# zachramsey/pm-rl

Hardware: AMD Instinct MI355X
Metric: env-steps/sec (whole node) at 65k envs x 30 assets; reward MAE vs CPU ref (higher is better)
Workload: dtype f64

## Files before the change

pm-rl_amd/csrc/step_relay.h:

```cpp
#pragma once
#include "env_step.h"
#include "scalar_vec.h"

namespace pmenv_dev {

struct RelayParams {
    uint32_t scal;
    uint32_t epoch;
    uint64_t* w;
    uint64_t* list;
    uint32_t* done;
    uint32_t spin;
    uint32_t rot;
    uint32_t grid;
    const int32_t* kp_in;
    int32_t* kp_out;
    const float* halo_in;
    float* halo_out;
    uint32_t* seq;
    int32_t* kp;
    float* halo;
    uint32_t B;
    uint32_t halo_stride;
    const float* obs;
    uint32_t par;
};
enum { kSeqD = 0, kSeqE = 1, kSeqV = 2, kSeqC = 3, kSeqEC = 4, kSeqHobs = 6 };

struct RelayCtx {
    uint32_t epoch;
    const int32_t* kp_in;
    int32_t* kp_out;
    const float* halo_in;
    float* halo_out;
};
template <bool SEQ>
__device__ __forceinline__ RelayCtx relay_ctx(const RelayParams& r) {
    RelayCtx c{r.epoch, r.kp_in, r.kp_out, r.halo_in, r.halo_out};
    if constexpr (SEQ) {
        const uint32_t par = __builtin_amdgcn_readfirstlane(r.seq[kSeqC]);
        c.epoch = __builtin_amdgcn_readfirstlane(r.seq[kSeqEC]);
        c.kp_in = r.kp + (size_t)par * r.B;
        c.kp_out = r.kp + (size_t)(par ^ 1u) * r.B;
        c.halo_in = r.halo + (size_t)par * r.halo_stride;
        c.halo_out = r.halo + (size_t)(par ^ 1u) * r.halo_stride;
    }
    return c;
}

struct KArgs {
    StepParams p;
    RelayParams r;
    uint32_t qtot;
};
__device__ __forceinline__ KArgs kargs() {
    typedef __attribute__((address_space(4))) const uint32_t KWord;
    KWord* ka = (KWord*)__builtin_amdgcn_kernarg_segment_ptr();
    asm volatile("" : "+s"(ka));
    uint32_t w[sizeof(KArgs) / 4];
#pragma unroll
    for (size_t i = 0; i < sizeof(KArgs) / 4; ++i) w[i] = ka[i];
    KArgs k;
    __builtin_memcpy(&k, w, sizeof(KArgs));
    return k;
}

constexpr uint32_t kStampSlots = 16, kStampMaxWg = 40960;
static __device__ uint64_t* g_relay_stamps;
template <bool ST, bool DRAIN = false>
__device__ __forceinline__ uint64_t relay_clock(uint32_t dep) {
    uint64_t t = 0;
    if constexpr (ST) {
        if constexpr (DRAIN)
            asm volatile("s_waitcnt vmcnt(0)\n\ts_memrealtime %0\n\ts_waitcnt lgkmcnt(0)" : "=s"(t) : "v"(dep) : "memory");
        else
            asm volatile("s_memrealtime %0\n\ts_waitcnt lgkmcnt(0)" : "=s"(t) : "v"(dep) : "memory");
    }
    return t;
}
template <bool ST, int K>
__device__ __forceinline__ void relay_stamps_put(uint32_t bid, uint32_t epoch, const uint64_t (&ts)[K]) {
    if constexpr (ST) {
        uint64_t* s = g_relay_stamps;
        if (s && threadIdx.x == 0 && bid < kStampMaxWg) {
#pragma unroll
            for (int k = 0; k < K; ++k) s[((size_t)(epoch % kStampSlots) * kStampMaxWg + bid) * 8 + k] = ts[k];
        }
    }
}

__device__ __forceinline__ void relay_put(uint64_t* w, uint32_t epoch, uint32_t bits) {
    __hip_atomic_store(w, ((uint64_t)epoch << 32) | bits, __ATOMIC_RELAXED, __HIP_MEMORY_SCOPE_AGENT);
}
__device__ __forceinline__ uint64_t relay_get(const uint64_t* w) {
    return __hip_atomic_load(const_cast<uint64_t*>(w), __ATOMIC_RELAXED, __HIP_MEMORY_SCOPE_AGENT);
}

__device__ __forceinline__ uint32_t relay_list_read(const RelayParams& r, uint32_t epoch) {
    __atomic_signal_fence(__ATOMIC_SEQ_CST);
    __builtin_amdgcn_s_waitcnt(0);
    __atomic_signal_fence(__ATOMIC_SEQ_CST);
    const uint64_t lw = relay_get(r.list);
    return (uint32_t)(lw >> 32) == epoch ? (uint32_t)lw : 0u;
}

template <int BLOCK, int KL, int KA, bool ST = false>
__device__ __forceinline__ uint32_t relay_scalar(const StepParams& p, const RelayParams& r, int s, uint32_t epoch,
                                                 int32_t* kp_out, uint64_t t_entry = 0) {
    uint64_t ts[3] = {t_entry, 0, 0};
    constexpr int EPW = 64 / KL, EPB = (BLOCK / 64) * EPW;
    const int lane = threadIdx.x & 63;
    const int b = s * EPB + (int)(threadIdx.x >> 6) * EPW + lane / KL;
    const int j = lane % KL;
    const int N = p.N;
    const bool env_ok = b < p.B;
    uint32_t listed;
    if constexpr (KA == 0) {
        const ScalarIn in = scalar_load<KL>(p, b, lane);
        const ScalarMid m = scalar_core<KL>(p, b, lane, in);
        if (env_ok && j < N) relay_put(r.w + (size_t)b * N + j, epoch, __float_as_uint(m.wp));
        if (env_ok && j == 0) kp_out[b] = m.k + 1;
        listed = relay_list_read(r, epoch);
        ts[1] = relay_clock<ST>(listed);
        scalar_tail<KL>(p, b, lane, in, m);
    } else {
        const VecIn<KA> in = vec_load<KL, KA, true>(p, b, lane);
        const VecMid<KA> m = vec_core<KL, KA, true>(p, b, lane, in);
#pragma unroll
        for (int e = 0; e < KA; ++e) {
            const int n = j + e * KL;
            if (env_ok && n < N) relay_put(r.w + (size_t)b * N + n, epoch, __float_as_uint(m.wp[e]));
        }
        if (env_ok && j == 0) kp_out[b] = in.k + 1;
        listed = relay_list_read(r, epoch);
        ts[1] = relay_clock<ST>(listed);
        vec_tail<KL, KA, true>(p, b, lane, in, m);
    }
    ts[2] = relay_clock<ST, true>(0);
    relay_stamps_put<ST>((uint32_t)s, epoch, ts);
    return listed;
}

template <int BLOCK, int V, int POL, bool OUT, bool ADOPT, bool ST = false>
__device__ __forceinline__ bool relay_tile(const StepParams& p, const RelayParams& r, uint32_t qtot, uint32_t spin, uint32_t t,
                                           uint32_t epoch, const int32_t* kp_in, const float* halo_in,
                                           float* halo_out, f4* sh4, f4* sh_bar, float* sh_wp, int32_t* sh_kc,
                                           int32_t* sh_ok, uint64_t t_entry = 0) {
    uint64_t ts[6] = {t_entry, 0, 0, 0, 0, 0};
    constexpr int kAux = POL == 1 ? 2 : 0;
    constexpr int CPW = BLOCK * V, F = 5;
    const int tid = threadIdx.x, lane = tid & 63, wave = tid >> 6;
    const uint32_t c0 = t * CPW;
    const uint32_t nblk = min((uint32_t)CPW, qtot - c0);
    const auto rs = make_rsrc(p.obs + (size_t)c0 * 4, nblk * 16u);
    f4 own[V];
#pragma unroll
    for (int v = 0; v < V; ++v) own[v] = buf_load4<kAux>(rs, (uint32_t)(64 * V * wave + 64 * v + lane) * 16u);
    const uint32_t ntiles = (qtot + CPW - 1) / CPW;
    const uint32_t nh = t + 1 < ntiles ? min(2u, qtot - c0 - nblk) : 0u;
    const float* hsrc = OUT ? p.obs + (size_t)(c0 + nblk) * 4 : halo_in + (size_t)t * 8;
    const f4 hal = buf_load4<0>(make_rsrc(hsrc, nh * 16u), tid < 2 ? (uint32_t)tid * 16u : 0xFFFFFFF0u);
    __builtin_amdgcn_sched_barrier(0);
    const int N = p.N, W = p.W, WF = W * F;
    const uint32_t per4 = (uint32_t)(N * WF) >> 2;
    const uint32_t b_lo = fdiv(c0, p.div_units);
    const uint32_t g_lo = b_lo * (uint32_t)N + fdiv(4u * (c0 - b_lo * per4), p.div_wf);
    const uint32_t ql = c0 + nblk - 1u;
    const uint32_t b_hi = fdiv(ql, p.div_units);
    const uint32_t g_hi = b_hi * (uint32_t)N + fdiv(4u * (ql - b_hi * per4) + 3u, p.div_wf);
    const bool mine = (uint32_t)tid <= g_hi - g_lo;
    const uint32_t g = g_lo + (mine ? (uint32_t)tid : 0u);
    const uint32_t b = g / (uint32_t)N, n = g - b * (uint32_t)N;
    const float* barb = env_bar(p, (int)b);
    const float nanv = __int_as_float(0x7fc00000);
    f4 xb = f4{nanv, nanv, nanv, nanv};
    int32_t kc = 0;
    uint64_t ww = 0;
    if (barb) xb = *reinterpret_cast<const f4*>(barb + (size_t)n * 4);
    kc = kp_in[b];
    ww = relay_get(r.w + g);
    bool ready = !mine || (uint32_t)(ww >> 32) == epoch;
    ts[1] = relay_clock<ST>((uint32_t)ww);
    for (uint32_t polls = 0; !ADOPT && !__all(ready) && polls < spin; ++polls) {
        __builtin_amdgcn_s_sleep(2);
        if (!ready) {
            ww = relay_get(r.w + g);
            ready = (uint32_t)(ww >> 32) == epoch;
        }
    }
    const bool wave_ok = __all(ready);
    ts[2] = relay_clock<ST>((uint32_t)ww);
    if (mine) {
        sh_bar[tid] = xb;
        sh_wp[tid] = __uint_as_float((uint32_t)ww);
        sh_kc[tid] = kc;
    }
#pragma unroll
    for (int v = 0; v < V; ++v) sh4[64 * V * wave + 64 * v + lane] = own[v];
    if (tid < 2) sh4[CPW + tid] = hal;
    if (lane == 0) sh_ok[wave] = wave_ok ? 1 : 0;
    __syncthreads();
    ts[3] = relay_clock<ST>(0);
    if constexpr (ADOPT) {
        bool tile_ok = true;
#pragma unroll
        for (int w = 0; w < BLOCK / 64; ++w) tile_ok = tile_ok && sh_ok[w] != 0;
        if (!tile_ok) return false;
        if (tid == 0)
            sh_ok[BLOCK / 64] = __hip_atomic_exchange(r.done + t, epoch, __ATOMIC_RELAXED, __HIP_MEMORY_SCOPE_AGENT) != epoch;
        __syncthreads();
        if (!sh_ok[BLOCK / 64]) return true;
    }
    const auto rd = OUT ? make_rsrc(p.obs_out + (size_t)c0 * 4, nblk * 16u) : rs;
    const bool first_out = !OUT && t > 0;
    bool ok = true;
#pragma unroll
    for (int v = 0; v < V; ++v) {
        const int j = 64 * V * wave + 64 * v + lane;
        const uint32_t q = min(c0 + (uint32_t)j, qtot - 1u);
        const uint32_t bq = fdiv(q, p.div_units);
        const uint32_t j0 = 4u * (q - bq * per4);
        const uint32_t row = fdiv(j0, p.div_wf);
        const int kk = (int)(j0 - row * (uint32_t)WF);
        const int i = (int)(bq * (uint32_t)N + row - g_lo);
        const f4 n1 = sh4[j + 1], n2 = sh4[j + 2];
        const float sh[4] = {n1.y, n1.z, n1.w, n2.x};
        const float un[4] = {own[v].x, own[v].y, own[v].z, own[v].w};
        f4 o = compose2(p, kk, sh_kc[i], un, sh, [&](f4& x, float& xwp) {
            x = sh_bar[i];
            xwp = sh_wp[i];
        });
        if (!ADOPT && v == 0) {
            int32_t okv = 1;
#pragma unroll
            for (int w = 0; w < BLOCK / 64; ++w) okv &= sh_ok[w];
            ok = __builtin_amdgcn_readfirstlane(okv) != 0;
        }
        buf_store4<kAux>(rd, ok ? (uint32_t)j * 16u : 0x80000000u, o);
        if (ok && first_out && j < 2) reinterpret_cast<f4*>(halo_out)[2 * (t - 1) + j] = o;
    }
    ts[4] = relay_clock<ST>(0);
    ts[5] = relay_clock<ST, true>(0);
    relay_stamps_put<ST>(r.scal + t, epoch, ts);
    return ok;
}

template <int BLOCK, int V, int POL, bool OUT, bool SEQ>
__device__ __forceinline__ void relay_adopt(f4* sh4, f4* sh_bar, float* sh_wp, int32_t* sh_kc, int32_t* sh_ok,
                                            uint32_t listed) {
    constexpr int kB = BLOCK / 64 + 1;
    const int wave = threadIdx.x >> 6;
    if ((threadIdx.x & 63) == 0) sh_ok[wave] = (int32_t)__builtin_amdgcn_readfirstlane(listed);
    __syncthreads();
    uint32_t n = 0;
#pragma unroll
    for (int w = 0; w < BLOCK / 64; ++w) n = max(n, (uint32_t)sh_ok[w]);
    if (n == 0) return;
    const KArgs ka = kargs();
    const RelayCtx c = relay_ctx<SEQ>(ka.r);
    for (uint32_t i = 0; i < n; ++i) {
        __syncthreads();
        if (threadIdx.x == 0) {
            const uint64_t e = relay_get(ka.r.list + 1 + i);
            int32_t t = (uint32_t)(e >> 32) == c.epoch ? (int32_t)(uint32_t)e : -1;
            if (t >= 0 && __hip_atomic_load(ka.r.done + t, __ATOMIC_RELAXED, __HIP_MEMORY_SCOPE_AGENT) == c.epoch)
                t = -1;
            sh_ok[kB] = t;
        }
        __syncthreads();
        const int32_t t = __builtin_amdgcn_readfirstlane(sh_ok[kB]);
        if (t >= 0)
            (void)relay_tile<BLOCK, V, POL, OUT, true>(ka.p, ka.r, ka.qtot, 0u, (uint32_t)t, c.epoch, c.kp_in, c.halo_in,
                                                       c.halo_out, sh4, sh_bar, sh_wp, sh_kc, sh_ok);
    }
}

template <int BLOCK, int V, int POL, bool OUT, bool SEQ>
__device__ __forceinline__ void relay_defer(uint32_t t, f4* sh4, f4* sh_bar, float* sh_wp, int32_t* sh_kc,
                                            int32_t* sh_ok) {
    const KArgs ka = kargs();
    const RelayCtx c = relay_ctx<SEQ>(ka.r);
    if (threadIdx.x == 0) {
        uint64_t lw = relay_get(ka.r.list), nw;
        do {
            nw = (uint32_t)(lw >> 32) == c.epoch ? lw + 1 : ((uint64_t)c.epoch << 32) | 1u;
        } while (!__hip_atomic_compare_exchange_strong(ka.r.list, &lw, nw, __ATOMIC_RELAXED, __ATOMIC_RELAXED,
                                                        __HIP_MEMORY_SCOPE_AGENT));
        const uint32_t slot = (uint32_t)(lw >> 32) == c.epoch ? (uint32_t)lw : 0u;
        relay_put(ka.r.list + 1 + slot, c.epoch, t);
        __atomic_signal_fence(__ATOMIC_SEQ_CST);
        __builtin_amdgcn_s_waitcnt(0);
        __atomic_signal_fence(__ATOMIC_SEQ_CST);
    }
    __syncthreads();
    (void)relay_tile<BLOCK, V, POL, OUT, true>(ka.p, ka.r, ka.qtot, 0u, t, c.epoch, c.kp_in, c.halo_in, c.halo_out, sh4,
                                               sh_bar, sh_wp, sh_kc, sh_ok);
}

template <int BLOCK, int V, int POL, bool OUT, int KL, int KA, int OCC = 1, bool SEQ = false, int ANY = 0>
__global__ __launch_bounds__(BLOCK) __attribute__((amdgpu_waves_per_eu(OCC))) void step_relay_kernel(
    StepParams p, RelayParams r, uint32_t qtot) {
    __shared__ f4 sh4[BLOCK * V + 2];
    __shared__ f4 sh_bar[BLOCK];
    __shared__ float sh_wp[BLOCK];
    __shared__ int32_t sh_kc[BLOCK];
    __shared__ int32_t sh_ok[BLOCK / 64 + 2];
    const RelayCtx c = relay_ctx<SEQ>(r);
    if constexpr (SEQ) {
        if (blockIdx.x == 0 && threadIdx.x == 0) {
            const uint64_t hobs = OUT ? 0ull : (uint64_t)(uintptr_t)r.obs;
            r.seq[kSeqD] = (uint32_t)((c.kp_in - r.kp) / r.B) ^ 1u;
            r.seq[kSeqE] = c.epoch;
            r.seq[kSeqV] = 1u;
            r.seq[kSeqHobs] = (uint32_t)hobs;
            r.seq[kSeqHobs + 1] = (uint32_t)(hobs >> 32);
        }
    }
    constexpr bool kSt = ANY == 2;
    const uint64_t t_entry = relay_clock<kSt>(0);
    uint32_t bid = blockIdx.x;
    if constexpr (ANY == 1) {
        bid += r.rot;
        if (bid >= r.grid) bid -= r.grid;
    }
    if (bid < r.scal) {
        const uint32_t listed = relay_scalar<BLOCK, KL, KA, kSt>(p, r, (int)bid, c.epoch, c.kp_out, t_entry);
        relay_adopt<BLOCK, V, POL, OUT, SEQ>(sh4, sh_bar, sh_wp, sh_kc, sh_ok, listed);
    } else if (!relay_tile<BLOCK, V, POL, OUT, false, kSt>(p, r, qtot, ANY == 1 ? r.spin : kRelaySpin, bid - r.scal, c.epoch,
                                                           c.kp_in, c.halo_in, c.halo_out, sh4, sh_bar, sh_wp, sh_kc,
                                                           sh_ok, t_entry)) {
        relay_defer<BLOCK, V, POL, OUT, SEQ>(bid - r.scal, sh4, sh_bar, sh_wp, sh_kc, sh_ok);
    }
}

static __global__ __launch_bounds__(256) void relay_prime_kernel(StepParams p, RelayParams r, int prime_kp, int seq) {
    uint32_t d = r.par;
    bool kp = prime_kp != 0, halo = p.halo != nullptr;
    if (seq) {
        d = __builtin_amdgcn_readfirstlane(r.seq[kSeqD]);
        const uint32_t e = __builtin_amdgcn_readfirstlane(r.seq[kSeqE]);
        const uint32_t v = __builtin_amdgcn_readfirstlane(r.seq[kSeqV]);
        const uint64_t hobs = (uint64_t)__builtin_amdgcn_readfirstlane(r.seq[kSeqHobs]) |
                              ((uint64_t)__builtin_amdgcn_readfirstlane(r.seq[kSeqHobs + 1]) << 32);
        kp = v == 0;
        halo = halo && (v == 0 || hobs != (uint64_t)(uintptr_t)p.obs);
        if (blockIdx.x == 0 && threadIdx.x == 0) {
            r.seq[kSeqC] = d;
            r.seq[kSeqEC] = e + 1u == 0u ? 1u : e + 1u;
        }
    }
    if (halo) {
        p.halo += (size_t)d * r.halo_stride;
        copy_halo(p);
    }
    if (kp) {
        int32_t* kpd = r.kp + (size_t)d * r.B;
        for (int b = blockIdx.x * blockDim.x + threadIdx.x; b < p.B; b += gridDim.x * blockDim.x) kpd[b] = p.k[b];
    }
}

}
```

Baseline: 104.5 million.

## Compose relay observation tiles via shared-memory image shift when rows share a mode

Each tile now votes on whether all its rows are in shift mode or full-ring mode, packing the mode bits with the readiness flag in the shared vote word. When the modes agree, the new bar and weight values are scattered into the shared-memory image, and each output chunk becomes a plain shifted read, or in full mode a phase-selected blend. This replaces the per-element division and compose2 call. Mixed tiles fall back to the old per-element path. It adds an extra __syncthreads and index arithmetic that is easy to get wrong.

```diff
diff --git a/pm-rl_amd/csrc/compose_shift.h b/pm-rl_amd/csrc/compose_shift.h
--- /dev/null
+++ b/pm-rl_amd/csrc/compose_shift.h
@@ -0,0 +1,33 @@
+#pragma once
+#include <stdint.h>
+
+#if defined(__HIPCC__)
+#define PMENV_SHIFT_HD __host__ __device__ inline
+#else
+#define PMENV_SHIFT_HD inline
+#endif
+
+namespace pmenv_shift {
+
+constexpr int kF = 5;
+enum { kModeShift = 1, kModeFull = 2 };
+
+PMENV_SHIFT_HD int32_t image_floats(int cpw) { return 4 * (cpw + 2); }
+PMENV_SHIFT_HD bool in_image(int32_t cell, int cpw) { return cell >= 0 && cell < image_floats(cpw); }
+
+PMENV_SHIFT_HD int row_mode(bool storage, int32_t k, int W) { return storage && k >= W - 1 ? kModeFull : kModeShift; }
+PMENV_SHIFT_HD bool rows_mixed(int votes) { return votes == (kModeShift | kModeFull); }
+
+PMENV_SHIFT_HD int32_t ring_slot(int32_t k, int W) { return (int32_t)(((uint32_t)k + 1u) % (uint32_t)W); }
+
+PMENV_SHIFT_HD int32_t src_cell(int32_t row_off, int WF, int e) { return row_off + WF + e; }
+PMENV_SHIFT_HD int32_t slot_cell(int32_t row_off, int32_t slot) { return row_off + slot * kF + (kF - 1); }
+
+PMENV_SHIFT_HD uint32_t chunk_phase(uint32_t q) { return (4u * (q % (uint32_t)kF)) % (uint32_t)kF; }
+PMENV_SHIFT_HD uint32_t phase_add(uint32_t phase, uint32_t chunks) {
+    const uint32_t s = phase + (4u * (chunks % (uint32_t)kF)) % (uint32_t)kF;
+    return s >= (uint32_t)kF ? s - (uint32_t)kF : s;
+}
+PMENV_SHIFT_HD int weight_elem(uint32_t phase) { return (kF - 1) - (int)phase; }
+
+}
diff --git a/pm-rl_amd/csrc/step_relay.h b/pm-rl_amd/csrc/step_relay.h
--- a/pm-rl_amd/csrc/step_relay.h
+++ b/pm-rl_amd/csrc/step_relay.h
@@ -1,8 +1,11 @@
 #pragma once
+#include "compose_shift.h"
 #include "env_step.h"
 #include "scalar_vec.h"
 
 namespace pmenv_dev {
+
+namespace ps = pmenv_shift;
 
 struct RelayParams {
     uint32_t scal;
@@ -190,6 +193,9 @@
     }
     const bool wave_ok = __all(ready);
     ts[2] = relay_clock<ST>((uint32_t)ww);
+    const int my_mode = ps::row_mode(p.ring_mode == PMENV_RING_STORAGE, kc, W);
+    const int wave_modes = (__any(mine && my_mode == ps::kModeShift) ? ps::kModeShift : 0) |
+                           (__any(mine && my_mode == ps::kModeFull) ? ps::kModeFull : 0);
     if (mine) {
         sh_bar[tid] = xb;
         sh_wp[tid] = __uint_as_float((uint32_t)ww);
@@ -198,14 +204,20 @@
 #pragma unroll
     for (int v = 0; v < V; ++v) sh4[64 * V * wave + 64 * v + lane] = own[v];
     if (tid < 2) sh4[CPW + tid] = hal;
-    if (lane == 0) sh_ok[wave] = wave_ok ? 1 : 0;
+    if (lane == 0) sh_ok[wave] = (wave_ok ? 1 : 0) | (wave_modes << 1);
     __syncthreads();
     ts[3] = relay_clock<ST>(0);
+    int32_t votes = -1, modes = 0;
+#pragma unroll
+    for (int w = 0; w < BLOCK / 64; ++w) {
+        const int32_t word = sh_ok[w];
+        votes &= word;
+        modes |= word;
+    }
+    const bool ok = __builtin_amdgcn_readfirstlane(votes & 1) != 0;
+    const int tile_modes = __builtin_amdgcn_readfirstlane(modes >> 1);
     if constexpr (ADOPT) {
-        bool tile_ok = true;
-#pragma unroll
-        for (int w = 0; w < BLOCK / 64; ++w) tile_ok = tile_ok && sh_ok[w] != 0;
-        if (!tile_ok) return false;
+        if (!ok) return false;
         if (tid == 0)
             sh_ok[BLOCK / 64] = __hip_atomic_exchange(r.done + t, epoch, __ATOMIC_RELAXED, __HIP_MEMORY_SCOPE_AGENT) != epoch;
         __syncthreads();
@@ -213,31 +225,69 @@
     }
     const auto rd = OUT ? make_rsrc(p.obs_out + (size_t)c0 * 4, nblk * 16u) : rs;
     const bool first_out = !OUT && t > 0;
-    bool ok = true;
-#pragma unroll
-    for (int v = 0; v < V; ++v) {
-        const int j = 64 * V * wave + 64 * v + lane;
-        const uint32_t q = min(c0 + (uint32_t)j, qtot - 1u);
-        const uint32_t bq = fdiv(q, p.div_units);
-        const uint32_t j0 = 4u * (q - bq * per4);
-        const uint32_t row = fdiv(j0, p.div_wf);
-        const int kk = (int)(j0 - row * (uint32_t)WF);
-        const int i = (int)(bq * (uint32_t)N + row - g_lo);
-        const f4 n1 = sh4[j + 1], n2 = sh4[j + 2];
-        const float sh[4] = {n1.y, n1.z, n1.w, n2.x};
-        const float un[4] = {own[v].x, own[v].y, own[v].z, own[v].w};
-        f4 o = compose2(p, kk, sh_kc[i], un, sh, [&](f4& x, float& xwp) {
-            x = sh_bar[i];
-            xwp = sh_wp[i];
-        });
-        if (!ADOPT && v == 0) {
-            int32_t okv = 1;
-#pragma unroll
-            for (int w = 0; w < BLOCK / 64; ++w) okv &= sh_ok[w];
-            ok = __builtin_amdgcn_readfirstlane(okv) != 0;
-        }
-        buf_store4<kAux>(rd, ok ? (uint32_t)j * 16u : 0x80000000u, o);
-        if (ok && first_out && j < 2) reinterpret_cast<f4*>(halo_out)[2 * (t - 1) + j] = o;
+    if (!ps::rows_mixed(tile_modes)) {
+        const bool full = tile_modes == ps::kModeFull;
+        float* img = reinterpret_cast<float*>(sh4);
+        if (mine) {
+            const int32_t row_off = (int32_t)(g_lo - b_lo * (uint32_t)N) * WF - (int32_t)(4u * (c0 - b_lo * per4)) + tid * WF;
+            const float wpv = __uint_as_float((uint32_t)ww);
+            const float src[5] = {xb.x, xb.y, xb.z, xb.w, wpv};
+#pragma unroll
+            for (int e = 0; e < F; ++e) {
+                const int32_t cell = ps::src_cell(row_off, WF, e);
+                if ((e < F - 1 || !full) && ps::in_image(cell, CPW)) img[cell] = src[e];
+            }
+            if (full) {
+                const int32_t slot = (int32_t)((uint32_t)(1 + kc) - fdiv((uint32_t)(1 + kc), p.div_w) * (uint32_t)W);
+                const int32_t cell = ps::slot_cell(row_off, slot);
+                if (ps::in_image(cell, CPW)) img[cell] = wpv;
+            }
+        }
+        __syncthreads();
+        const int j0 = 64 * V * wave + lane;
+        const uint32_t off0 = ok ? (uint32_t)j0 * 16u : 0x80000000u;
+        if (!full) {
+#pragma unroll
+            for (int v = 0; v < V; ++v) {
+                const int j = j0 + 64 * v;
+                const f4 n1 = sh4[j + 1], n2 = sh4[j + 2];
+                const f4 o = f4{n1.y, n1.z, n1.w, n2.x};
+                buf_store4<kAux>(rd, off0 + (uint32_t)v * 1024u, o);
+                if (ok && first_out && j < 2) reinterpret_cast<f4*>(halo_out)[2 * (t - 1) + j] = o;
+            }
+        } else {
+            uint32_t phase = ps::chunk_phase(c0 + (uint32_t)j0);
+#pragma unroll
+            for (int v = 0; v < V; ++v) {
+                const int j = j0 + 64 * v;
+                const f4 n0 = sh4[j], n1 = sh4[j + 1], n2 = sh4[j + 2];
+                const int we = ps::weight_elem(phase);
+                const f4 o = f4{we == 0 ? n0.x : n1.y, we == 1 ? n0.y : n1.z, we == 2 ? n0.z : n1.w, we == 3 ? n0.w : n2.x};
+                phase = ps::phase_add(phase, 64u);
+                buf_store4<kAux>(rd, off0 + (uint32_t)v * 1024u, o);
+                if (ok && first_out && j < 2) reinterpret_cast<f4*>(halo_out)[2 * (t - 1) + j] = o;
+            }
+        }
+    } else {
+#pragma unroll
+        for (int v = 0; v < V; ++v) {
+            const int j = 64 * V * wave + 64 * v + lane;
+            const uint32_t q = min(c0 + (uint32_t)j, qtot - 1u);
+            const uint32_t bq = fdiv(q, p.div_units);
+            const uint32_t j0 = 4u * (q - bq * per4);
+            const uint32_t row = fdiv(j0, p.div_wf);
+            const int kk = (int)(j0 - row * (uint32_t)WF);
+            const int i = (int)(bq * (uint32_t)N + row - g_lo);
+            const f4 n0 = sh4[j], n1 = sh4[j + 1], n2 = sh4[j + 2];
+            const float sh[4] = {n1.y, n1.z, n1.w, n2.x};
+            const float un[4] = {n0.x, n0.y, n0.z, n0.w};
+            f4 o = compose2(p, kk, sh_kc[i], un, sh, [&](f4& x, float& xwp) {
+                x = sh_bar[i];
+                xwp = sh_wp[i];
+            });
+            buf_store4<kAux>(rd, ok ? (uint32_t)j * 16u : 0x80000000u, o);
+            if (ok && first_out && j < 2) reinterpret_cast<f4*>(halo_out)[2 * (t - 1) + j] = o;
+        }
     }
     ts[4] = relay_clock<ST>(0);
     ts[5] = relay_clock<ST, true>(0);
```

New measurement: 103.3 million. 0.989x the previous value.
